# libjxl/libjxl

Hardware: AMD Instinct MI355X
Metric: Mpixels/s decode (VarDCT d1.0, 8K RGB) (higher is better)
Workload: dtype f32

## Files before the change

libjxl_amd/csrc/context.h:

```cpp
#pragma once
#include <stdint.h>
#include <stdio.h>
#include <string.h>

#include <algorithm>
#include <atomic>
#include <chrono>
#include <condition_variable>
#include <memory>
#include <mutex>
#include <vector>

#include "../../include/jxl_hip_codestream.h"
#include "../../include/jxl_hip_entropy.h"
#include "kernels.h"
#include "tile_bins.h"
#include "env_switches.h"

namespace jxlhip {

int Fail(jxlhip_ctx* c, int code, const char* fmt, ...);

#define HIPCHK(c, call)                                                              \
  do {                                                                               \
// ... 291 lines not shown
  int stage_state[kStageSlots] = {0};
  int stage_count = 0;
  int stage_cap = kStageSlots;
  PinnedBuf stage_chunk[kStageSlots / kStageChunk];
  size_t stage_bytes = 0;
  std::mutex stage_mu;
  std::condition_variable stage_cv;
  DevBuf<float> dc_tmp;
  DevBuf<uint8_t> dc_prec;
  DevBuf<uint8_t> host_frame_dev;
  PinnedBuf pinned_frame;
  DevBuf<float> alpha_dev;
  PinnedBuf alpha_host;
  DevBuf<int32_t> qdc_dev;
  StageState st;
  SlotState slots;
  float display_nits = 0.0f;
  uint32_t display_primaries = 0, display_white_point = 0;
  bool seq_open = false;
  uint64_t seq_expect = 0;
  bool generic_filters = false;
  int mfma = -1;
  int fuse = -1;
  DevBuf<uint2> cell_info;
  bool profiling = false;
  std::vector<ProfMarkRec> marks;
};

namespace jxlhip {

inline size_t SparseTableItems(const jxlhip_ctx* c) { return std::min(c->sp_off_host[0].bytes, c->sp_off_host[1].bytes) / 4; }

inline size_t OutSampleBytes(const jxlhip_output_format& o) {
  return o.sample_type == JXLHIP_SAMPLE_U8 ? 1 : (o.sample_type == JXLHIP_SAMPLE_F32 ? 4 : 2);
}
inline size_t OutPixelBytes(uint32_t kind, const jxlhip_output_format& o) {
  if (kind == JXLHIP_OUT_LINEAR_RGB_F32) return 12;
  return kind == JXLHIP_OUT_PACKED ? (size_t)o.num_channels * OutSampleBytes(o) : 0;
}
inline size_t OutPixelBytes(const jxlhip_ctx* c) { return OutPixelBytes(c->p.output_kind, c->p.out_format); }

inline size_t OutCols(const jxlhip_ctx* c) { return c->st.ups.factor > 1 ? c->st.ups.xsize : c->f.xsize; }
inline size_t OutRows(const jxlhip_ctx* c) { return c->st.ups.factor > 1 ? c->st.ups.ysize : c->f.y1 - c->f.y0; }
inline size_t BufCols(const jxlhip_ctx* c) { return c->st.blend.on ? c->st.blend.p.image_xsize : OutCols(c); }
inline size_t BufRows(const jxlhip_ctx* c) { return c->st.blend.on ? c->st.blend.p.image_ysize : OutRows(c); }

// ... 87 lines not shown
```

libjxl_amd/csrc/context.hip:

```cpp
#include <math.h>
#include <stdarg.h>
#include <stdlib.h>
#include <new>

#include "context.h"
#include "dither_pattern.inc"

extern "C" __attribute__((visibility("default"))) void jxlhip_debug_reload_env(void) {
  std::lock_guard<std::mutex> lock(jxlhip_env::g.mu);
  jxlhip_env::LoadLocked();
}

int jxlhip::Fail(jxlhip_ctx* c, int code, const char* fmt, ...) {
  if (c) {
    va_list ap;
    va_start(ap, fmt);
    vsnprintf(c->err, sizeof(c->err), fmt, ap);
    va_end(ap);
  }
  return code;
}

namespace {

// ... 69 lines not shown
  else free(c);
}

int jxlhip_create(int device, jxlhip_ctx** out) { return jxlhip_create_ex(device, nullptr, out); }

int jxlhip_create_ex(int device, const JxlMemoryManagerHip* memory_manager, jxlhip_ctx** out) {
  if (!out) return JXLHIP_ERR_INVALID_ARGUMENT;
  *out = nullptr;
  if (memory_manager && ((memory_manager->alloc == nullptr) != (memory_manager->free == nullptr)))
    return JXLHIP_ERR_INVALID_ARGUMENT;
  int ndev = 0;
  if (hipGetDeviceCount(&ndev) != hipSuccess || ndev <= 0) return JXLHIP_ERR_NO_DEVICE;
  if (device < 0 || device >= ndev) return JXLHIP_ERR_INVALID_ARGUMENT;
  jxlhip_ctx* c = NewCtx(memory_manager);
  if (!c) return JXLHIP_ERR_OUT_OF_MEMORY;
  c->device = device;
  {
    std::lock_guard<std::mutex> lock(jxlhip_env::g.mu);
    jxlhip_env::LoadLocked();
    const jxlhip_env::Switches& s = jxlhip_env::g;
    c->generic_filters = s.generic_filters.load();
    c->sparse_upload = s.sparse_upload.load();
    c->fuse = s.fuse.load();
    c->mfma = s.mfma.load();
    c->prepare_once = s.prepare_once.load();
    const int ss = s.stage_slots.load();
    if (ss != jxlhip_env::Switches::kUnset) {
      const int v = (ss + kStageChunk - 1) / kStageChunk * kStageChunk;
      c->stage_cap = v < kStageSlotsFirst ? kStageSlotsFirst : (v > kStageSlots ? kStageSlots : v);
    }
  }
  auto fail = [&](int code) {
    jxlhip_destroy(c);
    return code;
  };
  if (hipSetDevice(device) != hipSuccess) return fail(JXLHIP_ERR_HIP);
  if (c->own_stream.Create() != hipSuccess) return fail(JXLHIP_ERR_HIP);
  c->stream = c->own_stream;
  for (int i = 0; i < kPoolStreams; i++) {
    if (c->pool[i].Create() != hipSuccess || c->pool_ev[i].Create() != hipSuccess) return fail(JXLHIP_ERR_HIP);
  }
  if (c->frame_ev.Create() != hipSuccess) return fail(JXLHIP_ERR_HIP);
  if (c->counts.Reserve(c, (size_t)kCountStride * kCountBlocks) || c->error_flag.Reserve(c, 2) ||
      c->tables.Reserve(c, kTabFloats) || c->quant_enc.Reserve(c, JXLHIP_NUM_QUANT_TABLES))
    return fail(JXLHIP_ERR_OUT_OF_MEMORY);
  if (hipMemset(c->error_flag, 0, sizeof(int32_t) * 2) != hipSuccess ||
// ... 366 lines not shown
  if (!LaunchFiltersFast(f2, fp, 0, 2, (int)t.kind, c->stream))
    return Fail(c, JXLHIP_ERR_STATE, "EPF1 + EPF2 march refused a frame the EPF0 march accepted");
  return JXLHIP_OK;
}

int LaunchFiltersRows(jxlhip_ctx* c, const OutTarget& t, uint32_t fy0, uint32_t fy1, bool fused = false) {
  const FilterParams& fp = t.fp;
  DevFrame f = c->f;
  f.fy0 = fy0;
  f.fy1 = fy1;
  f.fused = fused ? 1u : 0u;
  f.cell_info = c->cell_info;
  ProfBegin(c);
  if (fused && c->p.lf.epf_iters == 3) {
    bool declined;
    const int rc = LaunchEpf0Then12(c, f, t, true, &declined);
    if (rc) return rc;
    if (declined) return Fail(c, JXLHIP_ERR_STATE, "fused EPF0 kernel refused a frame FusedEpf0Supported accepted");
    ProfMark(c, JXLHIP_KERNEL_FILTERS);
      HIPCHK(c, hipGetLastError());
    return JXLHIP_OK;
  }
  if (fused) {
    if (!LaunchFused(f, fp, (int)c->p.lf.gab, (int)c->p.lf.epf_iters, (int)t.kind, c->stream))
      return Fail(c, JXLHIP_ERR_STATE, "fused kernel refused a frame FusedSupported accepted");
    ProfMark(c, JXLHIP_KERNEL_FUSED);
      HIPCHK(c, hipGetLastError());
    return JXLHIP_OK;
  }
  bool fast = false;
  if (!c->generic_filters && fy1 > fy0 && c->p.lf.epf_iters == 3 && c->planes2) {
    bool declined;
    const int rc = LaunchEpf0Then12(c, f, t, false, &declined);
    if (rc) return rc;
    fast = !declined;
  } else if (!c->generic_filters && fy1 > fy0) {
    fast = LaunchFiltersFast(f, fp, (int)c->p.lf.gab, (int)c->p.lf.epf_iters, (int)t.kind, c->stream);
  }
  if (!fast && LaunchFilters(f, fp, (int)c->p.lf.gab, (int)c->p.lf.epf_iters, (int)t.kind, c->stream) != 0)
    return Fail(c, JXLHIP_ERR_INVALID_ARGUMENT, "unsupported filter configuration");
  ProfMark(c, JXLHIP_KERNEL_FILTERS);
  HIPCHK(c, hipGetLastError());
  return JXLHIP_OK;
}

bool WantFused(const jxlhip_ctx* c, uint32_t kind, const jxlhip_output_format& fmt) {
  const DevFrame& f = c->f;
// ... 479 lines not shown
```

libjxl_amd/csrc/entropy.cc:

```cpp
#include "env_switches.h"
#include <stdlib.h>
#include <string.h>
namespace jxlhip_env {
Switches g;
void LoadLocked() {
  g.wp_general.store(getenv("JXLHIP_WP_GENERAL") != nullptr);
  g.codestream_verbose.store(getenv("JXLHIP_CODESTREAM_VERBOSE") != nullptr);
  g.no_pipeline.store(getenv("JXLHIP_NO_PIPELINE") != nullptr);
  const char* e = getenv("JXLHIP_TEST_RANGE_GROUP");
  g.test_range_group.store(e ? atoll(e) : -1);
  const char* ife = getenv("JXLHIP_MULTI_INTERIOR_FIRST");
  g.multi_interior_first.store(!ife || atoi(ife) != 0 ? 1 : 0);
  auto num = [](const char* v, int unset) { return v ? atoi(v) : unset; };
  auto force = [](const char* v) { return v ? (atoi(v) != 0 ? 1 : 0) : -1; };
  g.fused_pc_rh.store(num(getenv("JXLHIP_FUSED_PC_RH"), 0));
  g.filter_rh.store(num(getenv("JXLHIP_FILTER_RH"), 0));
  g.big_wgs.store(num(getenv("JXLHIP_BIG_WGS"), Switches::kUnset));
  g.r_wgs.store(num(getenv("JXLHIP_R_WGS"), Switches::kUnset));
  g.multi_force_gather.store(getenv("JXLHIP_MULTI_FORCE_GATHER") != nullptr);
  const char* filters = getenv("JXLHIP_FILTERS");
  g.generic_filters.store(filters && !strcmp(filters, "generic"));
  g.sparse_upload.store(num(getenv("JXLHIP_SPARSE_UPLOAD"), 1) != 0);
  g.fuse.store(force(getenv("JXLHIP_FUSE")));
  g.mfma.store(force(getenv("JXLHIP_MFMA")));
  g.stage_slots.store(num(getenv("JXLHIP_STAGE_SLOTS"), Switches::kUnset));
  g.prepare_once.store(num(getenv("JXLHIP_PREPARE_ONCE"), 1) != 0);
  {
    const char* mp = getenv("JXLHIP_MAX_PIXELS");
    char* end = nullptr;
    const unsigned long long v = mp ? strtoull(mp, &end, 10) : 0ull;
    g.max_pixels.store((mp && end != mp && v != 0) ? v : (1ull << 30));
  }
  g.loaded.store(true, std::memory_order_release);
}
}
#include <math.h>
#include <stdlib.h>
#include <string.h>

#include <algorithm>
#include <functional>
#include <memory>
#include <mutex>
#include <new>
#include <vector>

// ... 2568 lines not shown
```

libjxl_amd/csrc/env_switches.h:

```cpp
#ifndef JXLHIP_ENV_SWITCHES_H_
#define JXLHIP_ENV_SWITCHES_H_
#include <atomic>
#include <mutex>

namespace jxlhip_env {
struct Switches {
  std::atomic<bool> loaded{false};
  std::atomic<bool> wp_general{false};
  std::atomic<bool> codestream_verbose{false};
  std::atomic<bool> no_pipeline{false};
  std::atomic<long long> test_range_group{-1};
  std::atomic<int> multi_interior_first{1};
  static constexpr int kUnset = -2147483647 - 1;
  std::atomic<int> fused_pc_rh{0};
  std::atomic<int> filter_rh{0};
  std::atomic<int> big_wgs{kUnset};
  std::atomic<int> r_wgs{kUnset};
  std::atomic<bool> multi_force_gather{false};
  std::atomic<unsigned long long> max_pixels{1ull << 30};
  std::atomic<bool> generic_filters{false};
  std::atomic<bool> sparse_upload{true};
  std::atomic<int> fuse{-1};
  std::atomic<int> mfma{-1};
  std::atomic<int> stage_slots{kUnset};
  std::atomic<bool> prepare_once{true};
  std::mutex mu;
};
extern Switches g;
void LoadLocked();
static inline const Switches& Get() {
  if (!g.loaded.load(std::memory_order_acquire)) {
    std::lock_guard<std::mutex> lock(g.mu);
    if (!g.loaded.load(std::memory_order_relaxed)) LoadLocked();
  }
  return g;
}
}
#endif
```

libjxl_amd/csrc/filters_march.h:

```cpp
#ifndef JXLHIP_FILTERS_MARCH_H_
#define JXLHIP_FILTERS_MARCH_H_

#include "dev_common.h"
#include "emit.h"
#include "kernels.h"

namespace jxlhip {
namespace {

__device__ __forceinline__ int MirrorF(int x, int n) {
  while (x < 0 || x >= n) x = x < 0 ? -x - 1 : 2 * n - 1 - x;
  return x;
}
__device__ __forceinline__ int Mirror1(int y, int n) {
  y = y < 0 ? -y - 1 : y;
  return y >= n ? 2 * n - 1 - y : y;
}

__device__ __forceinline__ uint32_t RowOffset(const DevFrame& f, int y) {
  const uint32_t ry = (uint32_t)(y - f.plane_y0);
  return (ry >> 3) * (f.tile_stride * 256u) + ((ry & 7u) << 5);
}

__device__ __forceinline__ float FromLeft(float v) {
// ... 34 lines not shown
  float y = __builtin_fabsf(d[0].y) * P.ch_scale[0];
  x = __builtin_fmaf(__builtin_fabsf(d[1].x), P.ch_scale[1], x);
  y = __builtin_fmaf(__builtin_fabsf(d[1].y), P.ch_scale[1], y);
  x = __builtin_fmaf(__builtin_fabsf(d[2].x), P.ch_scale[2], x);
  y = __builtin_fmaf(__builtin_fabsf(d[2].y), P.ch_scale[2], y);
  return v2f{Scalar(x), Scalar(y)};
}

__device__ __forceinline__ v2f AddLeftS(v2f acc, v2f p) {
  return v2f{Scalar(FromLeft(p.y) + acc.x), Scalar(acc.y + p.x)};
}
__device__ __forceinline__ v2f AddRightS(v2f acc, v2f p) {
  return v2f{Scalar(acc.x + p.y), Scalar(FromRight(p.x) + acc.y)};
}
__device__ __forceinline__ v2f FmaLeftS(v2f w, v2f p, v2f a) {
  float ax = a.x;
  asm("v_fmac_f32_dpp %0, %1, %2 wave_shr:1 row_mask:0xf bank_mask:0xf bound_ctrl:1" : "+v"(ax) : "v"(p.y), "v"(w.x));
  return v2f{ax, Scalar(__builtin_fmaf(w.y, p.x, a.y))};
}
__device__ __forceinline__ v2f FmaRightS(v2f w, v2f p, v2f a) {
  float ay = a.y;
  asm("v_fmac_f32_dpp %0, %1, %2 wave_shl:1 row_mask:0xf bank_mask:0xf bound_ctrl:1" : "+v"(ay) : "v"(p.x), "v"(w.y));
  return v2f{Scalar(__builtin_fmaf(w.x, p.y, a.x)), ay};
}

struct State {
  v2f x[3][8];
  v2f hs[3][4];
  v2f g[3][4];
  v2f du[4], dl[4];
  v2f pv[4], ph[4];
  v2f e[3][4];
  v2f dv[4];
};

struct Lane {
  uint32_t byte_off;
  bool sel0, sel1;
  int gx;
  bool out0, out1;
  v2f mul;
  v2f mul2;
  bool fix_left, fix_right_even, fix_right_odd;
  uint32_t sx4;
  uint32_t out_off;
  const float __attribute__((address_space(3))) * dither;
  const float __attribute__((address_space(3))) * slab;
};

enum RowSource : int { SRC_PLANES = 0, SRC_LDS = 1, SRC_LINEAR = 2 };
template <int SRC>
__device__ __forceinline__ uint32_t SrcRowOffset(const DevFrame& f, int y) {
  if constexpr (SRC == SRC_LINEAR) return (uint32_t)(y - f.plane_y0) * f.linear_stride;
  else return RowOffset(f, y);
}
static constexpr int kSlabCols = 128;
static constexpr int kSlabPlaneFloats = 8 * kSlabCols;
static constexpr int kSlabBytes = 3 * kSlabPlaneFloats * 4;

template <bool EDGE>
__device__ __forceinline__ v2f LdsPair(const Lane& L, int c, int row) {
  typedef v2f __attribute__((address_space(3))) * P2;
  const v2f v = *(P2)(L.slab + c * kSlabPlaneFloats + row * kSlabCols);
  if constexpr (!EDGE) return v;
  return v2f{L.sel0 ? v.y : v.x, L.sel1 ? v.y : v.x};
}

template <bool EDGE>
__device__ __forceinline__ v2f LoadPair(const char* rowp, Lane& L) {
  const v2f v = *(const v2f*)(rowp + L.byte_off);
  if constexpr (!EDGE) return v;
  return v2f{L.sel0 ? v.y : v.x, L.sel1 ? v.y : v.x};
}

typedef float f4u __attribute__((ext_vector_type(4), aligned(4)));
typedef float f2u __attribute__((ext_vector_type(2), aligned(4)));

struct XybConsts {
  v2f b01, b23, b45;
  v2f m0a, m1a, m2a;
};
// ... 114 lines not shown
    } else if (L.out1) {
      __builtin_nontemporal_store(o.p1.y, dst + 3);
      __builtin_nontemporal_store(o.p2.x, dst + 4);
      __builtin_nontemporal_store(o.p2.y, dst + 5);
    }
  } else {
    LaneOffset(L.out_off);
#pragma unroll
    for (int c = 0; c < 3; c++) {
      float* d = (float*)(out_row + (size_t)c * P.out_plane_stride * 4 + L.out_off);
      if (EDGE ? (L.out0 && L.out1) : L.out0) {
        __builtin_nontemporal_store(f2u{v[c].x, v[c].y}, (f2u*)d);
      } else if (!EDGE) {
      } else if (L.out0) {
        __builtin_nontemporal_store(v[c].x, d);
      } else if (L.out1) {
        __builtin_nontemporal_store(v[c].y, d + 1);
      }
    }
  }
}

enum StepKnown : int { kStepGeneric = 0, kStepInterior = 1, kStepEmit = 2, kStepFirst = 4 };
template <int GAB, int EPF, int OUTK, int FMT, int PH, bool EDGE, int SRC = SRC_PLANES, int KNOWN = kStepGeneric>
__device__ __forceinline__ void Step(State& s, int r, const DevFrame& f, const FilterParams& P,
                                     Lane& L, int prefetch_last_row, int y_begin, int y_end,
                                     float& inv_sigma_blk, float& inv_sigma_blk2, char* out_row, const XybConsts& K,
                                     int slab_y0 = 0, float sigma_pre = 0.0f, float sigma_prev = 0.0f) {
  constexpr int S0 = PH & 3, S1 = (PH + 3) & 3, S2 = (PH + 2) & 3;
  constexpr int X0 = PH & 7, X1 = (PH + 7) & 7, X2 = (PH + 6) & 7, X3 = (PH + 5) & 7;
  const int H = (int)f.ysize;
  if constexpr (SRC == SRC_LDS) {
    if constexpr (PH < 7) {
      const int nrow = (KNOWN & kStepInterior) ? PH + 1 : Mirror1(r + 1, H) - slab_y0;
#pragma unroll
      for (int c = 0; c < 3; c++) s.x[c][(PH + 1) & 7] = LdsPair<EDGE>(L, c, nrow);
    }
  } else if constexpr (PH % kBurst == 0) {
    LaneOffset(L.byte_off);
#pragma unroll
    for (int b = 0; b < kBurst; b++) {
      int pr = r + kAhead + b;
      pr = pr > prefetch_last_row ? prefetch_last_row : pr;
      const uint32_t off = SrcRowOffset<SRC>(f, Mirror1(pr, H));
#pragma unroll
      for (int c = 0; c < 3; c++) s.x[c][(PH + kAhead + b) & 7] = LoadPair<EDGE>((const char*)f.xyb[c] + off, L);
    }
  }
  v2f gq[3];
  if constexpr (GAB) {
#pragma unroll
    for (int c = 0; c < 3; c++) {
      const v2f cur = s.x[c][X0];
      s.hs[c][S0] = v2f{Scalar(FromLeft(cur.y) + cur.y), Scalar(FromRight(cur.x) + cur.x)};
      const v2f sum1 = s.hs[c][S1] + (s.x[c][X2] + cur);
      const v2f sum2 = s.hs[c][S2] + s.hs[c][S0];
      gq[c] = Fma2(sum2, P.gab_w[c][2], Fma2(sum1, P.gab_w[c][1], s.x[c][X1] * P.gab_w[c][0]));
    }
  } else {
#pragma unroll
    for (int c = 0; c < 3; c++) gq[c] = s.x[c][X0];
  }
  constexpr int Q0 = GAB ? S1 : S0;
  constexpr int Q1 = (Q0 + 3) & 3, Q2 = (Q0 + 2) & 3, Q3 = (Q0 + 1) & 3;
  const int q = GAB ? r - 1 : r;
  v2f gq1[3], gq2[3], gq3[3];
#pragma unroll
  for (int c = 0; c < 3; c++) {
    gq1[c] = GAB ? s.g[c][Q1] : s.x[c][X1];
    gq2[c] = GAB ? s.g[c][Q2] : s.x[c][X2];
    gq3[c] = GAB ? s.g[c][Q3] : s.x[c][X3];
  }
  v2f outv[3];
  int o;
  if constexpr (EPF) {
    {
      v2f dvert[3], dhor[3];
#pragma unroll
      for (int c = 0; c < 3; c++) {
        dvert[c] = gq1[c] - gq[c];
        dhor[c] = v2f{Scalar(FromLeft(gq[c].y) - gq[c].x), Scalar(gq[c].x - gq[c].y)};
        if constexpr (GAB) s.g[c][Q0] = gq[c];
      }
      s.du[Q0] = AbsScaleSum(dvert, P);
      s.dl[Q0] = AbsScaleSum(dhor, P);
    }
    {
      const v2f du_c = s.du[Q1], dl_c = s.dl[Q1];
      v2f v = AddLeftS(s.du[Q2], du_c);
      v = v + du_c;
      v = AddRightS(v, du_c);
      s.pv[Q1] = v + s.du[Q0];
      v2f h = AddLeftS(s.dl[Q2], dl_c);
      h = h + dl_c;
      h = AddRightS(h, dl_c);
      s.ph[Q1] = h + s.dl[Q0];
    }
    o = q - 2;
    const float kMinSigma = -3.90524291751269967465540850526868f;
    constexpr bool kInt = (KNOWN & kStepInterior) != 0;
    static_assert(!kInt || SRC == SRC_LDS, "kStepInterior: the fused kernel's march");
    constexpr int kIy = (PH - GAB - 2 + 16) & 7;
    if (kInt ? (kIy == 0 || (EPF == 2 && (KNOWN & kStepFirst) && kIy == 7)) : ((o & 7) == 0 || o == y_begin - (EPF == 2 ? 1 : 0))) {
      float is = (kInt ? kIy == 0 : (o & 7) == 0) ? sigma_pre : sigma_prev;
      if constexpr (SRC != SRC_LDS) {
// ... 103 lines not shown
```

libjxl_amd/csrc/fused_pc.h:

```cpp
#ifndef JXLHIP_FUSED_PC_H_
#define JXLHIP_FUSED_PC_H_

#include <stdlib.h>

#include <type_traits>

#include "blocks_common.h"
#include "env_switches.h"
#include "filters_march.h"

static constexpr int kProducerPrio = 3;

namespace jxlhip {

namespace {

typedef __attribute__((address_space(3))) float LdsF;
typedef __attribute__((address_space(3))) uint32_t LdsU;

static constexpr int kFusedHalo = 8;
static constexpr int kFusedUse = kSlabCols - 2 * kFusedHalo;

typedef const DevFrame __attribute__((address_space(4))) * FrameArgs;
__device__ __forceinline__ FrameArgs Fresh(FrameArgs q) {
// ... 250 lines not shown
#pragma unroll
  for (int c = 0; c < 3; c++) {
    k.coef[c] = (const char*)f->coeffs[c];
    k.dc[c] = (const char*)f->dc[c];
    k.xyb[c] = f->xyb[c];
  }
  k.cell_info = (const char*)f->cell_info;
  k.inv_sigma = (const char*)f->inv_sigma;
  k.xsb = (int)f->xsb;
  k.tile_stride = f->tile_stride;
  k.plane_tile_row0 = f->plane_y0 >> 3;
  k.inv_global_scale = f->inv_global_scale;
  k.x_dm = f->x_dm;
  k.b_dm = f->b_dm;
  k.cfl_base_x = f->cfl_base_x;
  k.cfl_base_b = f->cfl_base_b;
  k.color_scale = f->color_scale;
#pragma unroll
  for (int i = 0; i < 4; i++) k.bias[i] = f->biases[i];
  return k;
}
__device__ __forceinline__ u4v AsmLoad4S(const char* base, uint32_t off) {
  u4v r;
  asm volatile("global_load_dwordx4 %0, %1, %2" : "=v"(r) : "v"(off), "s"(base) : "memory");
  return r;
}
__device__ __forceinline__ u2v AsmLoad2S(const char* base, uint32_t off) {
  u2v r;
  asm volatile("global_load_dwordx2 %0, %1, %2" : "=v"(r) : "v"(off), "s"(base) : "memory");
  return r;
}
__device__ __forceinline__ uint32_t AsmLoad1S(const char* base, uint32_t off) {
  uint32_t r;
  asm volatile("global_load_dword %0, %1, %2" : "=v"(r) : "v"(off), "s"(base) : "memory");
  return r;
}

__device__ __forceinline__ void PcLanded(PcNext& n) { asm volatile("" : "+v"(n.ci), "+v"(n.sg)); }
__device__ __forceinline__ void PcLanded(PcGroupRegs& R) {
#pragma unroll
  for (int s = 0; s < 2; s++)
#pragma unroll
    for (int c = 0; c < 3; c++) asm volatile("" : "+v"(R.st[s].rows[c]), "+v"(R.st[s].dcv[c]));
}

__device__ __forceinline__ void PcRequest(const PcK& K, PcNext& n, int nb, int bc0) {
  const int lane = threadIdx.x & 63;
  int col = bc0 + (lane & 15);
  col = col < 0 ? 0 : (col >= K.xsb ? K.xsb - 1 : col);
  const uint32_t cell = (uint32_t)(nb * K.xsb + col);
  n.nb = nb;
  n.ci = AsmLoad2S(K.cell_info, cell * 8u);
  n.sg = AsmLoad1S(K.inv_sigma, cell * 4u);
}

__device__ __forceinline__ void PcIssue(const PcK& K, LdsU* list, const PcNext& n, int bc0, PcGroupRegs& R) {
  const int lane = threadIdx.x & 63;
// ... 93 lines not shown
          const float sc = c == 0 ? sx : sb;
          const float cc = c == 0 ? x_cc : b_cc;
          unpack(T.rows[c], q);
#pragma unroll
          for (int k = 0; k < 8; k++) {
            const float d = AdjustQuantBias(q[k], c == 0 ? bias0 : bias2, bias3) * (tab[c][k] * sc);
            v[k] = __builtin_fmaf(cc, vy[k], d);
          }
        }
        if (j == 0) v[0] = __uint_as_float(T.dcv[c]);
        IdctReg<8>(v);
        Transpose8Lanes(v, bit3);
        IdctReg<8>(v);
        LdsF* dst = slab + c * kSlabPlaneFloats + j * kSlabCols + T.cell * 8;
        if (valid) {
          *(P4)dst = f4v{v[0], v[1], v[2], v[3]};
          *(P4)(dst + 4) = f4v{v[4], v[5], v[6], v[7]};
        }
      }
    }
  }
}

template <int HX>
__device__ __forceinline__ void ProducePC2(FrameArgs fa, StripLds* w, int bc0, int y_begin, int y_end, int nb_last) {
  const int lane = threadIdx.x & 63;
  const int r_first = HX ? y_begin - 8 : y_begin;
  const int G = PcGroups<HX>(y_begin, y_end);
  const PcK K = MakePcK(fa);
  float tab[3][8];
  {
    const int j = lane >> 3;
#pragma unroll
    for (int c = 0; c < 3; c++) {
      const float4 t0 = *(const float4*)(fa->dequant + c * 64 + j * 8);
      const float4 t1 = *(const float4*)(fa->dequant + c * 64 + j * 8 + 4);
      tab[c][0] = t0.x, tab[c][1] = t0.y, tab[c][2] = t0.z, tab[c][3] = t0.w;
      tab[c][4] = t1.x, tab[c][5] = t1.y, tab[c][6] = t1.z, tab[c][7] = t1.w;
    }
  }
  LdsU* list = (LdsU*)w->list[0];
  auto group_nb = [&](int g) { return GroupBlockRow(r_first + 8 * (g < G ? g : G - 1), nb_last); };
  PcGroupRegs A, B;
  PcNext n0, n1;
  uint32_t sg_a = 0, sg_b = 0;
  PcRequest(K, n0, group_nb(0), bc0);
  asm volatile("s_waitcnt vmcnt(0)" ::: "memory");
  PcLanded(n0);
  PcIssue(K, list, n0, bc0, A);
  sg_a = n0.sg;
  PcRequest(K, n1, group_nb(1), bc0);
  asm volatile("s_waitcnt vmcnt(0)" ::: "memory");
  PcLanded(A);
  PcLanded(n1);
  auto body = [&](int g, PcGroupRegs& CUR, PcGroupRegs& NXT, uint32_t& sg_cur, uint32_t& sg_nxt, PcNext& nn) {
    LdsF* slab = (LdsF*)w->slab[(g & 1)];
    PcDmaPlanes(K, slab, CUR.mp, CUR.nb, bc0);
    PcIssue(K, list, nn, bc0, NXT);
    sg_nxt = nn.sg;
    PcRequest(K, nn, group_nb(g + 2), bc0);
    PcDecode(K, slab, CUR, tab);
    if (lane < 16) ((LdsU*)w->sigma[g & 1])[lane] = sg_cur;
    PcBarrierProducer();
    PcLanded(NXT);
    PcLanded(nn);
  };
  for (int g = 0; g < G; g += 2) {
    body(g, A, B, sg_a, sg_b, n1);
    if (g + 1 < G) body(g + 1, B, A, sg_b, sg_a, n1);
  }
}

int FusedRowsPC(unsigned strips, unsigned rows, unsigned per_cu = kPcPerCu) {
  const int forced = jxlhip_env::Get().fused_pc_rh.load(std::memory_order_relaxed);
  if (forced > 0) return (forced + 7) & ~7;
  return ChunkRows(strips, rows, DeviceCus() * per_cu, 16, 1024, 8, 6 + 16);
}

}
}
#endif
```

libjxl_amd/csrc/kernels.h:

```cpp
#ifndef JXLHIP_KERNELS_H_
#define JXLHIP_KERNELS_H_

#include "dev_common.h"

namespace jxlhip {

struct WorkLists {
  WorkItem* list[kNumClasses];
  uint32_t* count;
};

struct SharpLut {
  float v[8];
};

struct FilterParams {
  float gab_w[3][3];
  float ch_scale[3];
  float sm[3], bsm[3];
  float opsin_bias[3];
  float cbrt_bias[3];
  float minv[9];
  float xyb_bias[6];
  float mcol[3][4];
// ... 14 lines not shown
                   const SharpLut& lut, hipStream_t st);
void LaunchBlocks(const DevFrame& f, const WorkLists& wl, uint32_t cells, const float* wc,
                  const float* resample, hipStream_t st, const FilterParams* emit = nullptr);
int LaunchFilters(const DevFrame& f, const FilterParams& p, int gab, int epf_iters,
                  int output_kind, hipStream_t st);

bool LaunchFiltersFast(const DevFrame& f, const FilterParams& p, int gab, int epf_iters,
                       int output_kind, hipStream_t st);
bool FastFixedFormat(const jxlhip_output_format& o);

bool LaunchEpf0(const DevFrame& f, const FilterParams& p, int gab, float* const dst[3], hipStream_t st);

void LaunchExpandSparse(const uint8_t* sparse, const uint32_t* offsets, int16_t* dense, uint32_t g0, uint32_t n, hipStream_t st);

bool LaunchOrient(const void* src, size_t src_stride, uint32_t xsize, uint32_t ysize, uint32_t bytes_per_pixel,
                  uint32_t orientation, void* dst, size_t dst_stride, hipStream_t st);

void MfmaDct32Constants(float* host );
void MfmaDct16Constants(float* host );
void LaunchMfma32(const DevFrame& f, const WorkLists& wl, uint32_t cells, hipStream_t st, const FilterParams* emit = nullptr);
void LaunchMfma16(const DevFrame& f, const WorkLists& wl, uint32_t cells, hipStream_t st);

bool FusedSupported(const DevFrame& f, int gab, int epf_iters, int output_kind);
bool LaunchFused(const DevFrame& f, const FilterParams& p, int gab, int epf_iters, int output_kind,
                 hipStream_t st);
bool FusedEpf0Supported(const DevFrame& f, int gab);
bool LaunchFusedEpf0(const DevFrame& f, const FilterParams& p, int gab, float* const dst[3], hipStream_t st);
unsigned DeviceCus();
inline int ChunkRows(unsigned wgx, unsigned rows, unsigned resident, int first, int last, int step, int overhead) {
  int best = 64;
  double best_cost = 1e30;
  for (int rh = first; rh <= last; rh += step) {
    const unsigned wgs = wgx * ((rows + rh - 1) / rh);
    const unsigned gens = (wgs + resident - 1) / resident;
    const double cost = (double)gens * (rh + overhead);
    if (cost < best_cost) {
      best_cost = cost;
      best = rh;
    }
  }
  return best;
}

constexpr uint32_t kNoiseSegFills = 128;
constexpr uint32_t kNoiseSegs = (3u * 256u * 16u + kNoiseSegFills - 1) / kNoiseSegFills;
constexpr uint32_t kNoiseJumpWords = 128 * 4;
struct NoiseArgs {
// ... 144 lines not shown
```

libjxl_amd/csrc/kernels_fused.hip:

```cpp
#include "fused_pc.h"

namespace jxlhip {

namespace {

template <int GAB, int EPF, int OUTK, int FMT, bool EDGE, bool INTERIOR, int NB = 2>
__device__ __forceinline__ void MarchPC(const DevFrame& f, const FilterParams& P, Lane& L, StripLdsT<NB>* w, int bc0,
                                        int y_begin, int y_end) {
  constexpr int HX = MarchGeom<GAB, EPF>::HX;
  constexpr int KI = INTERIOR ? (int)kStepInterior : 0;
  constexpr int KE = INTERIOR ? (int)(kStepInterior | kStepEmit) : 0;
  constexpr int KF = INTERIOR ? (int)kStepFirst : 0;
  const int H = (int)f.ysize;
  const int r_first = HX ? y_begin - 8 : y_begin;
  const int r_last = y_end + HX - 1;
  const int nb_last = (H - 1) >> 3;
  const int G = PcGroups<HX>(y_begin, y_end);
  State s;
#pragma unroll
  for (int k = 0; k < 8; k++)
#pragma unroll
    for (int c = 0; c < 3; c++) s.x[c][k] = v2f{0.0f, 0.0f};
#pragma unroll
  for (int k = 0; k < 4; k++) {
#pragma unroll
    for (int c = 0; c < 3; c++) {
      s.hs[c][k] = v2f{0.0f, 0.0f};
      s.g[c][k] = v2f{0.0f, 0.0f};
      s.e[c][k] = v2f{0.0f, 0.0f};
    }
    s.du[k] = v2f{0.0f, 0.0f};
    s.dl[k] = v2f{0.0f, 0.0f};
    s.pv[k] = v2f{0.0f, 0.0f};
    s.ph[k] = v2f{0.0f, 0.0f};
    s.dv[k] = v2f{0.0f, 0.0f};
  }
  float inv_sigma_blk = -1.0f, inv_sigma_blk2 = -1.0f;
  float sigma_last = -1.0f;
  const XybConsts KC = MakeXybConsts(P);
  const size_t out_row_bytes = OUTK == JXLHIP_OUT_XYB_PLANAR ? P.out_stride * 4 : P.out_stride;
  char* out_row = (char*)P.out + (ptrdiff_t)(r_first - HX - (int)f.y0) * (ptrdiff_t)out_row_bytes;
  const float __attribute__((address_space(3)))* const slab0 = L.slab;
  const LdsF* sig0 = (const LdsF*)w->sigma[0] + ((int)(L.sx4 >> 2) - bc0);
  int i = 0;
  auto enter_group = [&](int g) -> float {
    const int b = NB == 2 ? (g & 1) : g % NB;
    L.slab = slab0 + b * (3 * kSlabPlaneFloats);
    return EPF ? sig0[b * 16] : 0.0f;
  };
#define JXLHIP_PSTEPK(K, KN)                                                                                          \
  Step<GAB, EPF, OUTK, FMT, K, EDGE, SRC_LDS, KN>(s, r + K, f, P, L, 0, y_begin, y_end, inv_sigma_blk,         \
                                                  inv_sigma_blk2, out_row, KC, slab_y0, sigma_pre, sigma_prev);       \
  out_row += out_row_bytes
#define JXLHIP_PGROUP(KLOW, KHIGH)                                                       \
  {                                                                                      \
    const int slab_y0 = GroupBlockRow(r, nb_last) * 8;                                   \
    const float sigma_prev = sigma_last;                                                 \
    const float sigma_pre = enter_group(i);                                              \
    sigma_last = sigma_pre;                                                              \
    {                                                                                    \
      const int row0 = INTERIOR ? 0 : Mirror1(r, H) - slab_y0;                           \
      _Pragma("unroll") for (int c = 0; c < 3; c++) s.x[c][0] = LdsPair<EDGE>(L, c, row0); \
    }                                                                                    \
    JXLHIP_PSTEPK(0, (0 < HX ? (KLOW) : (KHIGH)));                                       \
    JXLHIP_PSTEPK(1, (1 < HX ? (KLOW) : (KHIGH)));                                       \
    JXLHIP_PSTEPK(2, (2 < HX ? (KLOW) : (KHIGH)));                                       \
    JXLHIP_PSTEPK(3, (3 < HX ? (KLOW) : (KHIGH)));                                       \
    JXLHIP_PSTEPK(4, (KHIGH));                                                           \
    JXLHIP_PSTEPK(5, (KHIGH));                                                           \
    JXLHIP_PSTEPK(6, (KHIGH));                                                           \
    JXLHIP_PSTEPK(7, (KHIGH));                                                           \
    i++;                                                                                 \
  }
  PcBarrierMarch();
  if constexpr (HX > 0) {
    const int r = r_first;
    const int slab_y0 = GroupBlockRow(r, nb_last) * 8;
    const float sigma_prev = sigma_last;
    const float sigma_pre = enter_group(i);
    sigma_last = sigma_pre;
    {
      const int row0 = INTERIOR ? 8 - HX : Mirror1(r + 8 - HX, H) - slab_y0;
#pragma unroll
      for (int c = 0; c < 3; c++) s.x[c][8 - HX] = LdsPair<EDGE>(L, c, row0);
    }
    out_row += (8 - HX) * out_row_bytes;
    if constexpr (HX >= 4) { JXLHIP_PSTEPK(4, KI); }
    if constexpr (HX >= 3) { JXLHIP_PSTEPK(5, KI); }
    if constexpr (HX >= 2) { JXLHIP_PSTEPK(6, KI); }
    JXLHIP_PSTEPK(7, KI);
    i++;
    PcBarrierMarch();
  }
  int r = HX ? y_begin : r_first;
  if constexpr (INTERIOR) {
    JXLHIP_PGROUP(KI | KF, KE | KF)
    if (i < G) PcBarrierMarch();
    for (r += 8; r < y_end; r += 8) {
      JXLHIP_PGROUP(KE, KE)
      if (i < G) PcBarrierMarch();
    }
  } else {
    for (; r_last - r >= HX; r += 8) {
      JXLHIP_PGROUP(0, 0)
      if (i < G) PcBarrierMarch();
    }
  }
  if (HX > 0 && (INTERIOR || r <= r_last)) {
    const int slab_y0 = GroupBlockRow(r, nb_last) * 8;
    const float sigma_prev = sigma_last;
    const float sigma_pre = enter_group(i);
    sigma_last = sigma_pre;
    {
      const int row0 = INTERIOR ? 0 : Mirror1(r, H) - slab_y0;
#pragma unroll
      for (int c = 0; c < 3; c++) s.x[c][0] = LdsPair<EDGE>(L, c, row0);
    }
    JXLHIP_PSTEPK(0, KE);
    if constexpr (HX >= 2) { JXLHIP_PSTEPK(1, KE); }
    if constexpr (HX >= 3) { JXLHIP_PSTEPK(2, KE); }
    if constexpr (HX >= 4) { JXLHIP_PSTEPK(3, KE); }
  }
#undef JXLHIP_PGROUP
#undef JXLHIP_PSTEPK
}

template <int GAB, int EPF, int OUTK, int FMT, typename CT>
__global__ __launch_bounds__(128, kPcWaves) void k_fused_pc(DevFrame f, FilterParams P, int RH, int strips, int nwg) {
  __shared__ StripLds lds;
  const int lane = threadIdx.x & 63;
  const int wave = (int)(threadIdx.x >> 6);
  const float __attribute__((address_space(3)))* dither_lds = nullptr;
  if constexpr (OUTK == JXLHIP_OUT_PACKED) {
    __shared__ float s_dither[1024];
    if (P.fmt.sample_type == JXLHIP_SAMPLE_U8) {
      for (int i = threadIdx.x; i < 1024; i += 128) s_dither[i] = P.dither[i];
      __syncthreads();
    }
    dither_lds = (const float __attribute__((address_space(3)))*)s_dither;
  }
  const int per = (int)gridDim.x >> 3;
  const int logical = ((int)blockIdx.x & 7) * per + ((int)blockIdx.x >> 3);
  if (logical >= nwg) return;
  const int strip = logical % strips, chunk = logical / strips;
  const int W = (int)f.xsize;
  const int x_first = strip * kFusedUse;
  const int y_begin = (int)f.fy0 + chunk * RH;
  const int y_end = min(y_begin + RH, (int)f.fy1);
  if (x_first >= W || y_begin >= y_end) return;
  const int x0 = x_first - kFusedHalo;
  const int bc0 = x0 >> 3;
  const FrameArgs fa = (FrameArgs)__builtin_amdgcn_kernarg_segment_ptr();
  if (wave == 1) {
    __builtin_amdgcn_s_setprio(kProducerPrio);
    if constexpr (sizeof(CT) == 2) ProducePC2<MarchGeom<GAB, EPF>::HX>(fa, &lds, bc0, y_begin, y_end, ((int)f.ysize - 1) >> 3);
    else
      ProducePC<MarchGeom<GAB, EPF>::HX, CT>(fa, &lds, bc0, y_begin, y_end, ((int)f.ysize - 1) >> 3);
    return;
  }
  Lane L;
  L.gx = x0 + 2 * lane;
  L.dither = dither_lds;
  const int m0 = MirrorF(L.gx, W), m1 = MirrorF(L.gx + 1, W);
  int base = (m0 & ~1) - x0;
  base = base < 0 ? 0 : (base > kSlabCols - 2 ? kSlabCols - 2 : base);
  L.sel0 = m0 & 1;
  L.sel1 = m1 & 1;
  L.byte_off = 0;
  L.slab = (const float __attribute__((address_space(3)))*)lds.slab[0] + base;
  const bool edge = x0 < 0 || x0 + kSlabCols > W;
  const bool lane_in = lane >= kFusedHalo / 2 && lane < 64 - kFusedHalo / 2;
  L.out0 = lane_in && L.gx < W;
  L.out1 = lane_in && L.gx + 1 < W;
  const int gxc = L.gx < 0 ? 0 : (L.gx >= W ? W - 1 : L.gx);
  L.sx4 = (uint32_t)(gxc >> 3) * 4u;
  L.out_off = (uint32_t)(L.gx < 0 ? 0 : L.gx) * (OUTK == JXLHIP_OUT_LINEAR_RGB_F32 ? 12u : 4u);
  const int ix = gxc & 7;
  L.mul = v2f{ix == 0 ? P.bsm[1] : P.sm[1], ix == 6 ? P.bsm[1] : P.sm[1]};
  L.mul2 = v2f{ix == 0 ? P.bsm[2] : P.sm[2], ix == 6 ? P.bsm[2] : P.sm[2]};
  L.fix_left = L.gx == -2;
  L.fix_right_even = L.gx == W;
  L.fix_right_odd = L.gx == W - 1;
  const bool interior = (y_begin & 7) == 0 && ((y_end - y_begin) & 7) == 0 && y_begin >= 8 &&
                        y_end + 8 <= (int)f.ysize;
  if (interior) {
    if (edge) MarchPC<GAB, EPF, OUTK, FMT, true, true>(f, P, L, &lds, bc0, y_begin, y_end);
    else MarchPC<GAB, EPF, OUTK, FMT, false, true>(f, P, L, &lds, bc0, y_begin, y_end);
  } else {
    if (edge) MarchPC<GAB, EPF, OUTK, FMT, true, false>(f, P, L, &lds, bc0, y_begin, y_end);
    else MarchPC<GAB, EPF, OUTK, FMT, false, false>(f, P, L, &lds, bc0, y_begin, y_end);
  }
}

template <int GAB, int EPF, int OUTK, int FMT = -1>
void LaunchFusedPcT(const DevFrame& f, const FilterParams& p, hipStream_t st) {
  const unsigned strips = (f.xsize + kFusedUse - 1) / kFusedUse;
  const int RH = FusedRowsPC(strips, f.fy1 - f.fy0);
  const unsigned nwg = strips * ((f.fy1 - f.fy0 + RH - 1) / RH);
  const dim3 grid((nwg + 7) & ~7u);
  if (f.coeff_type == JXLHIP_COEFF_I16)
    hipLaunchKernelGGL((k_fused_pc<GAB, EPF, OUTK, FMT, int16_t>), grid, dim3(128), 0, st, f, p, RH, (int)strips, (int)nwg);
  else
    hipLaunchKernelGGL((k_fused_pc<GAB, EPF, OUTK, FMT, int32_t>), grid, dim3(128), 0, st, f, p, RH, (int)strips, (int)nwg);
}

}

bool FusedSupported(const DevFrame& f, int gab, int epf_iters, int output_kind) {
  (void)gab;
  if (epf_iters > 2) return false;
  if (output_kind == JXLHIP_OUT_PACKED) return false;
  if (f.xsize < 16 || f.ysize < 16) return false;
  const uint32_t tail = f.ysize & 7u;
  if (tail >= 1 && tail <= 3) return false;
  if ((f.fy0 & 7u) != 0) return false;
  if ((uint64_t)f.plane_tile_rows * f.tile_stride * 256u >= (1ull << 32)) return false;
  if ((uint64_t)f.xsg * f.ysg * f.coef_stride64 * 64u * (f.coeff_type == JXLHIP_COEFF_I16 ? 2u : 4u) >= (1ull << 32)) return false;
  return true;
}

bool LaunchFused(const DevFrame& f, const FilterParams& p, int gab, int epf_iters, int output_kind, hipStream_t st) {
  if (!FusedSupported(f, gab, epf_iters, output_kind)) return false;
#define JXLHIP_FUSED_PCX(G, E)                                    \
  if (gab == G && epf_iters == E) {                               \
    if (output_kind == 0) LaunchFusedPcT<G, E, 0>(f, p, st);      \
    else LaunchFusedPcT<G, E, 1>(f, p, st);                       \
    return true;                                                  \
  }
  JXLHIP_FUSED_PCX(1, 1)
  JXLHIP_FUSED_PCX(0, 0)
  JXLHIP_FUSED_PCX(0, 1)
  JXLHIP_FUSED_PCX(1, 0)
  JXLHIP_FUSED_PCX(0, 2)
  JXLHIP_FUSED_PCX(1, 2)
#undef JXLHIP_FUSED_PCX
  return false;
}

}
```

Before: 121,300.

## Add opt-in producer-side Gaborish pass in fused PC kernel; pad global loads with s_nop

Adds an env-gated mode (JXLHIP_FUSED_PREGAB, off by default) in which the producer wave applies the Gaborish smoothing to each decoded slab in LDS, so the consumer march skips its own Gaborish work and reads pre-filtered rows with a remapped slab index. This is meant to move filter arithmetic off the consumer wave and onto the producer, at the cost of an extra full vmcnt wait and LDS rewrites in the producer. Separately, every inline-asm global load in the fused producer now starts with an s_nop 4, which changes instruction timing on the default path as well.

```diff
diff --git a/libjxl_amd/csrc/context.h b/libjxl_amd/csrc/context.h
--- a/libjxl_amd/csrc/context.h
+++ b/libjxl_amd/csrc/context.h
@@ -337,6 +337,7 @@
   bool generic_filters = false;
   int mfma = -1;
   int fuse = -1;
+  int fused_pregab = -1;
   DevBuf<uint2> cell_info;
   bool profiling = false;
   std::vector<ProfMarkRec> marks;
diff --git a/libjxl_amd/csrc/context.hip b/libjxl_amd/csrc/context.hip
--- a/libjxl_amd/csrc/context.hip
+++ b/libjxl_amd/csrc/context.hip
@@ -115,6 +115,7 @@
     c->generic_filters = s.generic_filters.load();
     c->sparse_upload = s.sparse_upload.load();
     c->fuse = s.fuse.load();
+    c->fused_pregab = s.fused_pregab.load();
     c->mfma = s.mfma.load();
     c->prepare_once = s.prepare_once.load();
     const int ss = s.stage_slots.load();
@@ -527,7 +528,7 @@
     return JXLHIP_OK;
   }
   if (fused) {
-    if (!LaunchFused(f, fp, (int)c->p.lf.gab, (int)c->p.lf.epf_iters, (int)t.kind, c->stream))
+    if (!LaunchFused(f, fp, (int)c->p.lf.gab, (int)c->p.lf.epf_iters, (int)t.kind, c->fused_pregab, c->stream))
       return Fail(c, JXLHIP_ERR_STATE, "fused kernel refused a frame FusedSupported accepted");
     ProfMark(c, JXLHIP_KERNEL_FUSED);
       HIPCHK(c, hipGetLastError());
diff --git a/libjxl_amd/csrc/entropy.cc b/libjxl_amd/csrc/entropy.cc
--- a/libjxl_amd/csrc/entropy.cc
+++ b/libjxl_amd/csrc/entropy.cc
@@ -22,6 +22,7 @@
   g.generic_filters.store(filters && !strcmp(filters, "generic"));
   g.sparse_upload.store(num(getenv("JXLHIP_SPARSE_UPLOAD"), 1) != 0);
   g.fuse.store(force(getenv("JXLHIP_FUSE")));
+  g.fused_pregab.store(force(getenv("JXLHIP_FUSED_PREGAB")));
   g.mfma.store(force(getenv("JXLHIP_MFMA")));
   g.stage_slots.store(num(getenv("JXLHIP_STAGE_SLOTS"), Switches::kUnset));
   g.prepare_once.store(num(getenv("JXLHIP_PREPARE_ONCE"), 1) != 0);
diff --git a/libjxl_amd/csrc/env_switches.h b/libjxl_amd/csrc/env_switches.h
--- a/libjxl_amd/csrc/env_switches.h
+++ b/libjxl_amd/csrc/env_switches.h
@@ -21,6 +21,7 @@
   std::atomic<bool> generic_filters{false};
   std::atomic<bool> sparse_upload{true};
   std::atomic<int> fuse{-1};
+  std::atomic<int> fused_pregab{-1};
   std::atomic<int> mfma{-1};
   std::atomic<int> stage_slots{kUnset};
   std::atomic<bool> prepare_once{true};
diff --git a/libjxl_amd/csrc/filters_march.h b/libjxl_amd/csrc/filters_march.h
--- a/libjxl_amd/csrc/filters_march.h
+++ b/libjxl_amd/csrc/filters_march.h
@@ -80,6 +80,16 @@
   float ay = a.y;
   asm("v_fmac_f32_dpp %0, %1, %2 wave_shl:1 row_mask:0xf bank_mask:0xf bound_ctrl:1" : "+v"(ay) : "v"(p.x), "v"(w.y));
   return v2f{Scalar(__builtin_fmaf(w.x, p.y, a.x)), ay};
+}
+
+__device__ __forceinline__ v2f GabHs(v2f cur) {
+  return v2f{Scalar(FromLeft(cur.y) + cur.y), Scalar(FromRight(cur.x) + cur.x)};
+}
+__device__ __forceinline__ v2f GabRow(v2f above, v2f centre, v2f below, v2f hs_above, v2f hs_centre, v2f hs_below,
+                                      const float* w) {
+  const v2f sum1 = hs_centre + (above + below);
+  const v2f sum2 = hs_above + hs_below;
+  return Fma2(sum2, w[2], Fma2(sum1, w[1], centre * w[0]));
 }
 
 struct State {
@@ -115,6 +125,12 @@
 static constexpr int kSlabCols = 128;
 static constexpr int kSlabPlaneFloats = 8 * kSlabCols;
 static constexpr int kSlabBytes = 3 * kSlabPlaneFloats * 4;
+
+template <int PREGAB>
+__device__ __forceinline__ int SlabRowOfStep(int r, int H, int slab_y0) {
+  if constexpr (PREGAB) return (Mirror1(r - 1, H) + 1 - slab_y0) & 7;
+  else return Mirror1(r, H) - slab_y0;
+}
 
 template <bool EDGE>
 __device__ __forceinline__ v2f LdsPair(const Lane& L, int c, int row) {
@@ -275,17 +291,19 @@
 }
 
 enum StepKnown : int { kStepGeneric = 0, kStepInterior = 1, kStepEmit = 2, kStepFirst = 4 };
-template <int GAB, int EPF, int OUTK, int FMT, int PH, bool EDGE, int SRC = SRC_PLANES, int KNOWN = kStepGeneric>
+template <int GAB, int EPF, int OUTK, int FMT, int PH, bool EDGE, int SRC = SRC_PLANES, int KNOWN = kStepGeneric,
+          int PREGAB = 0>
 __device__ __forceinline__ void Step(State& s, int r, const DevFrame& f, const FilterParams& P,
                                      Lane& L, int prefetch_last_row, int y_begin, int y_end,
                                      float& inv_sigma_blk, float& inv_sigma_blk2, char* out_row, const XybConsts& K,
                                      int slab_y0 = 0, float sigma_pre = 0.0f, float sigma_prev = 0.0f) {
   constexpr int S0 = PH & 3, S1 = (PH + 3) & 3, S2 = (PH + 2) & 3;
   constexpr int X0 = PH & 7, X1 = (PH + 7) & 7, X2 = (PH + 6) & 7, X3 = (PH + 5) & 7;
+  static_assert(!PREGAB || (GAB && SRC == SRC_LDS), "PREGAB: Gaborish applied by the fused kernel's producing wave");
   const int H = (int)f.ysize;
   if constexpr (SRC == SRC_LDS) {
     if constexpr (PH < 7) {
-      const int nrow = (KNOWN & kStepInterior) ? PH + 1 : Mirror1(r + 1, H) - slab_y0;
+      const int nrow = (KNOWN & kStepInterior) ? PH + 1 : SlabRowOfStep<PREGAB>(r + 1, H, slab_y0);
 #pragma unroll
       for (int c = 0; c < 3; c++) s.x[c][(PH + 1) & 7] = LdsPair<EDGE>(L, c, nrow);
     }
@@ -301,14 +319,11 @@
     }
   }
   v2f gq[3];
-  if constexpr (GAB) {
+  if constexpr (GAB && !PREGAB) {
 #pragma unroll
     for (int c = 0; c < 3; c++) {
-      const v2f cur = s.x[c][X0];
-      s.hs[c][S0] = v2f{Scalar(FromLeft(cur.y) + cur.y), Scalar(FromRight(cur.x) + cur.x)};
-      const v2f sum1 = s.hs[c][S1] + (s.x[c][X2] + cur);
-      const v2f sum2 = s.hs[c][S2] + s.hs[c][S0];
-      gq[c] = Fma2(sum2, P.gab_w[c][2], Fma2(sum1, P.gab_w[c][1], s.x[c][X1] * P.gab_w[c][0]));
+      s.hs[c][S0] = GabHs(s.x[c][X0]);
+      gq[c] = GabRow(s.x[c][X2], s.x[c][X1], s.x[c][X0], s.hs[c][S2], s.hs[c][S1], s.hs[c][S0], P.gab_w[c]);
     }
   } else {
 #pragma unroll
@@ -320,9 +335,9 @@
   v2f gq1[3], gq2[3], gq3[3];
 #pragma unroll
   for (int c = 0; c < 3; c++) {
-    gq1[c] = GAB ? s.g[c][Q1] : s.x[c][X1];
-    gq2[c] = GAB ? s.g[c][Q2] : s.x[c][X2];
-    gq3[c] = GAB ? s.g[c][Q3] : s.x[c][X3];
+    gq1[c] = (GAB && !PREGAB) ? s.g[c][Q1] : s.x[c][X1];
+    gq2[c] = (GAB && !PREGAB) ? s.g[c][Q2] : s.x[c][X2];
+    gq3[c] = (GAB && !PREGAB) ? s.g[c][Q3] : s.x[c][X3];
   }
   v2f outv[3];
   int o;
@@ -333,7 +348,7 @@
       for (int c = 0; c < 3; c++) {
         dvert[c] = gq1[c] - gq[c];
         dhor[c] = v2f{Scalar(FromLeft(gq[c].y) - gq[c].x), Scalar(gq[c].x - gq[c].y)};
-        if constexpr (GAB) s.g[c][Q0] = gq[c];
+        if constexpr (GAB && !PREGAB) s.g[c][Q0] = gq[c];
       }
       s.du[Q0] = AbsScaleSum(dvert, P);
       s.dl[Q0] = AbsScaleSum(dhor, P);
diff --git a/libjxl_amd/csrc/fused_pc.h b/libjxl_amd/csrc/fused_pc.h
--- a/libjxl_amd/csrc/fused_pc.h
+++ b/libjxl_amd/csrc/fused_pc.h
@@ -296,17 +296,17 @@
 }
 __device__ __forceinline__ u4v AsmLoad4S(const char* base, uint32_t off) {
   u4v r;
-  asm volatile("global_load_dwordx4 %0, %1, %2" : "=v"(r) : "v"(off), "s"(base) : "memory");
+  asm volatile("s_nop 4\n\tglobal_load_dwordx4 %0, %1, %2" : "=v"(r) : "v"(off), "s"(base) : "memory");
   return r;
 }
 __device__ __forceinline__ u2v AsmLoad2S(const char* base, uint32_t off) {
   u2v r;
-  asm volatile("global_load_dwordx2 %0, %1, %2" : "=v"(r) : "v"(off), "s"(base) : "memory");
+  asm volatile("s_nop 4\n\tglobal_load_dwordx2 %0, %1, %2" : "=v"(r) : "v"(off), "s"(base) : "memory");
   return r;
 }
 __device__ __forceinline__ uint32_t AsmLoad1S(const char* base, uint32_t off) {
   uint32_t r;
-  asm volatile("global_load_dword %0, %1, %2" : "=v"(r) : "v"(off), "s"(base) : "memory");
+  asm volatile("s_nop 4\n\tglobal_load_dword %0, %1, %2" : "=v"(r) : "v"(off), "s"(base) : "memory");
   return r;
 }
 
@@ -446,8 +446,56 @@
   }
 }
 
-template <int HX>
-__device__ __forceinline__ void ProducePC2(FrameArgs fa, StripLds* w, int bc0, int y_begin, int y_end, int nb_last) {
+template <bool EDGE>
+__device__ __forceinline__ void GabPass(const FilterParams& P, const Lane& L0, int buffer, int nb, int rows, bool refill,
+                                        v2f (&up2)[3], v2f (&up1)[3]) {
+  Lane L;
+  L.slab = L0.slab + buffer * (3 * kSlabPlaneFloats);
+  L.sel0 = L0.sel0, L.sel1 = L0.sel1;
+  L.out0 = L0.out0, L.out1 = L0.out1;
+  v2f hs2[3], hs1[3];
+#pragma unroll
+  for (int c = 0; c < 3; c++) {
+    hs2[c] = GabHs(up2[c]);
+    hs1[c] = GabHs(up1[c]);
+  }
+#pragma unroll
+  for (int k = 0; k < 8; k++) {
+    v2f cur[3];
+#pragma unroll
+    for (int c = 0; c < 3; c++) cur[c] = k < rows ? LdsPair<EDGE>(L, c, k) : up1[c];
+    if (k == 0 && nb == 0) {
+#pragma unroll
+      for (int c = 0; c < 3; c++) {
+        up1[c] = cur[c];
+        hs1[c] = GabHs(cur[c]);
+      }
+    }
+#pragma unroll
+    for (int c = 0; c < 3; c++) {
+      const v2f below = (k == 0 && refill) ? up1[c] : cur[c];
+      const v2f hs0 = GabHs(below);
+      const v2f g = GabRow(up2[c], up1[c], below, hs2[c], hs1[c], hs0, P.gab_w[c]);
+      typedef v2f __attribute__((address_space(3))) * P2;
+      LdsF* dst = (LdsF*)L.slab + c * kSlabPlaneFloats + k * kSlabCols;
+      if constexpr (!EDGE) {
+        *(P2)dst = g;
+      } else if (L.out1) {
+        *(P2)dst = g;
+      } else if (L.out0) {
+        *dst = g.x;
+      }
+      up2[c] = up1[c];
+      hs2[c] = hs1[c];
+      up1[c] = cur[c];
+      hs1[c] = (k == 0 && refill) ? GabHs(cur[c]) : hs0;
+    }
+  }
+}
+
+template <int HX, int PREGAB = 0, bool EDGE = false>
+__device__ __forceinline__ void ProducePC2(FrameArgs fa, StripLds* w, int bc0, int y_begin, int y_end, int nb_last,
+                                           const FilterParams* P = nullptr, const Lane* L = nullptr) {
   const int lane = threadIdx.x & 63;
   const int r_first = HX ? y_begin - 8 : y_begin;
   const int G = PcGroups<HX>(y_begin, y_end);
@@ -468,6 +516,9 @@
   PcGroupRegs A, B;
   PcNext n0, n1;
   uint32_t sg_a = 0, sg_b = 0;
+  v2f up2[3] = {v2f{0.0f, 0.0f}, v2f{0.0f, 0.0f}, v2f{0.0f, 0.0f}}, up1[3] = {v2f{0.0f, 0.0f}, v2f{0.0f, 0.0f}, v2f{0.0f, 0.0f}};
+  int nb_prev = -1;
+  const int H = PREGAB ? (int)fa->ysize : 0;
   PcRequest(K, n0, group_nb(0), bc0);
   asm volatile("s_waitcnt vmcnt(0)" ::: "memory");
   PcLanded(n0);
@@ -484,6 +535,11 @@
     sg_nxt = nn.sg;
     PcRequest(K, nn, group_nb(g + 2), bc0);
     PcDecode(K, slab, CUR, tab);
+    if constexpr (PREGAB) {
+      asm volatile("s_waitcnt vmcnt(0)" ::: "memory");
+      GabPass<EDGE>(*P, *L, g & 1, CUR.nb, H - 8 * CUR.nb, CUR.nb == nb_prev && CUR.nb == nb_last, up2, up1);
+      nb_prev = CUR.nb;
+    }
     if (lane < 16) ((LdsU*)w->sigma[g & 1])[lane] = sg_cur;
     PcBarrierProducer();
     PcLanded(NXT);
diff --git a/libjxl_amd/csrc/kernels.h b/libjxl_amd/csrc/kernels.h
--- a/libjxl_amd/csrc/kernels.h
+++ b/libjxl_amd/csrc/kernels.h
@@ -60,7 +60,7 @@
 void LaunchMfma16(const DevFrame& f, const WorkLists& wl, uint32_t cells, hipStream_t st);
 
 bool FusedSupported(const DevFrame& f, int gab, int epf_iters, int output_kind);
-bool LaunchFused(const DevFrame& f, const FilterParams& p, int gab, int epf_iters, int output_kind,
+bool LaunchFused(const DevFrame& f, const FilterParams& p, int gab, int epf_iters, int output_kind, int pregab,
                  hipStream_t st);
 bool FusedEpf0Supported(const DevFrame& f, int gab);
 bool LaunchFusedEpf0(const DevFrame& f, const FilterParams& p, int gab, float* const dst[3], hipStream_t st);
diff --git a/libjxl_amd/csrc/kernels_fused.hip b/libjxl_amd/csrc/kernels_fused.hip
--- a/libjxl_amd/csrc/kernels_fused.hip
+++ b/libjxl_amd/csrc/kernels_fused.hip
@@ -4,7 +4,7 @@
 
 namespace {
 
-template <int GAB, int EPF, int OUTK, int FMT, bool EDGE, bool INTERIOR, int NB = 2>
+template <int GAB, int EPF, int OUTK, int FMT, bool EDGE, bool INTERIOR, int PREGAB = 0, int NB = 2>
 __device__ __forceinline__ void MarchPC(const DevFrame& f, const FilterParams& P, Lane& L, StripLdsT<NB>* w, int bc0,
                                         int y_begin, int y_end) {
   constexpr int HX = MarchGeom<GAB, EPF>::HX;
@@ -49,7 +49,7 @@
     return EPF ? sig0[b * 16] : 0.0f;
   };
 #define JXLHIP_PSTEPK(K, KN)                                                                                          \
-  Step<GAB, EPF, OUTK, FMT, K, EDGE, SRC_LDS, KN>(s, r + K, f, P, L, 0, y_begin, y_end, inv_sigma_blk,         \
+  Step<GAB, EPF, OUTK, FMT, K, EDGE, SRC_LDS, KN, PREGAB>(s, r + K, f, P, L, 0, y_begin, y_end, inv_sigma_blk,         \
                                                   inv_sigma_blk2, out_row, KC, slab_y0, sigma_pre, sigma_prev);       \
   out_row += out_row_bytes
 #define JXLHIP_PGROUP(KLOW, KHIGH)                                                       \
@@ -59,7 +59,7 @@
     const float sigma_pre = enter_group(i);                                              \
     sigma_last = sigma_pre;                                                              \
     {                                                                                    \
-      const int row0 = INTERIOR ? 0 : Mirror1(r, H) - slab_y0;                           \
+      const int row0 = INTERIOR ? 0 : SlabRowOfStep<PREGAB>(r, H, slab_y0);              \
       _Pragma("unroll") for (int c = 0; c < 3; c++) s.x[c][0] = LdsPair<EDGE>(L, c, row0); \
     }                                                                                    \
     JXLHIP_PSTEPK(0, (0 < HX ? (KLOW) : (KHIGH)));                                       \
@@ -80,7 +80,7 @@
     const float sigma_pre = enter_group(i);
     sigma_last = sigma_pre;
     {
-      const int row0 = INTERIOR ? 8 - HX : Mirror1(r + 8 - HX, H) - slab_y0;
+      const int row0 = INTERIOR ? 8 - HX : SlabRowOfStep<PREGAB>(r + 8 - HX, H, slab_y0);
 #pragma unroll
       for (int c = 0; c < 3; c++) s.x[c][8 - HX] = LdsPair<EDGE>(L, c, row0);
     }
@@ -112,7 +112,7 @@
     const float sigma_pre = enter_group(i);
     sigma_last = sigma_pre;
     {
-      const int row0 = INTERIOR ? 0 : Mirror1(r, H) - slab_y0;
+      const int row0 = INTERIOR ? 0 : SlabRowOfStep<PREGAB>(r, H, slab_y0);
 #pragma unroll
       for (int c = 0; c < 3; c++) s.x[c][0] = LdsPair<EDGE>(L, c, row0);
     }
@@ -125,8 +125,9 @@
 #undef JXLHIP_PSTEPK
 }
 
-template <int GAB, int EPF, int OUTK, int FMT, typename CT>
+template <int GAB, int EPF, int OUTK, int FMT, typename CT, int PREGAB = 0>
 __global__ __launch_bounds__(128, kPcWaves) void k_fused_pc(DevFrame f, FilterParams P, int RH, int strips, int nwg) {
+  static_assert(!PREGAB || (GAB && sizeof(CT) == 2), "PREGAB: a Gaborish stage list on the pipelined producer");
   __shared__ StripLds lds;
   const int lane = threadIdx.x & 63;
   const int wave = (int)(threadIdx.x >> 6);
@@ -151,24 +152,33 @@
   const int x0 = x_first - kFusedHalo;
   const int bc0 = x0 >> 3;
   const FrameArgs fa = (FrameArgs)__builtin_amdgcn_kernarg_segment_ptr();
-  if (wave == 1) {
-    __builtin_amdgcn_s_setprio(kProducerPrio);
-    if constexpr (sizeof(CT) == 2) ProducePC2<MarchGeom<GAB, EPF>::HX>(fa, &lds, bc0, y_begin, y_end, ((int)f.ysize - 1) >> 3);
-    else
-      ProducePC<MarchGeom<GAB, EPF>::HX, CT>(fa, &lds, bc0, y_begin, y_end, ((int)f.ysize - 1) >> 3);
-    return;
-  }
   Lane L;
   L.gx = x0 + 2 * lane;
-  L.dither = dither_lds;
   const int m0 = MirrorF(L.gx, W), m1 = MirrorF(L.gx + 1, W);
   int base = (m0 & ~1) - x0;
   base = base < 0 ? 0 : (base > kSlabCols - 2 ? kSlabCols - 2 : base);
   L.sel0 = m0 & 1;
   L.sel1 = m1 & 1;
-  L.byte_off = 0;
   L.slab = (const float __attribute__((address_space(3)))*)lds.slab[0] + base;
   const bool edge = x0 < 0 || x0 + kSlabCols > W;
+  if (wave == 1) {
+    __builtin_amdgcn_s_setprio(kProducerPrio);
+    constexpr int HX = MarchGeom<GAB, EPF>::HX;
+    const int nb_last = ((int)f.ysize - 1) >> 3;
+    if constexpr (PREGAB) {
+      L.out0 = L.gx >= 0 && L.gx < W;
+      L.out1 = L.gx >= 0 && L.gx + 1 < W;
+      if (edge) ProducePC2<HX, 1, true>(fa, &lds, bc0, y_begin, y_end, nb_last, &P, &L);
+      else ProducePC2<HX, 1, false>(fa, &lds, bc0, y_begin, y_end, nb_last, &P, &L);
+    } else if constexpr (sizeof(CT) == 2) {
+      ProducePC2<HX>(fa, &lds, bc0, y_begin, y_end, nb_last);
+    } else {
+      ProducePC<HX, CT>(fa, &lds, bc0, y_begin, y_end, nb_last);
+    }
+    return;
+  }
+  L.dither = dither_lds;
+  L.byte_off = 0;
   const bool lane_in = lane >= kFusedHalo / 2 && lane < 64 - kFusedHalo / 2;
   L.out0 = lane_in && L.gx < W;
   L.out1 = lane_in && L.gx + 1 < W;
@@ -184,20 +194,26 @@
   const bool interior = (y_begin & 7) == 0 && ((y_end - y_begin) & 7) == 0 && y_begin >= 8 &&
                         y_end + 8 <= (int)f.ysize;
   if (interior) {
-    if (edge) MarchPC<GAB, EPF, OUTK, FMT, true, true>(f, P, L, &lds, bc0, y_begin, y_end);
-    else MarchPC<GAB, EPF, OUTK, FMT, false, true>(f, P, L, &lds, bc0, y_begin, y_end);
+    if (edge) MarchPC<GAB, EPF, OUTK, FMT, true, true, PREGAB>(f, P, L, &lds, bc0, y_begin, y_end);
+    else MarchPC<GAB, EPF, OUTK, FMT, false, true, PREGAB>(f, P, L, &lds, bc0, y_begin, y_end);
   } else {
-    if (edge) MarchPC<GAB, EPF, OUTK, FMT, true, false>(f, P, L, &lds, bc0, y_begin, y_end);
-    else MarchPC<GAB, EPF, OUTK, FMT, false, false>(f, P, L, &lds, bc0, y_begin, y_end);
+    if (edge) MarchPC<GAB, EPF, OUTK, FMT, true, false, PREGAB>(f, P, L, &lds, bc0, y_begin, y_end);
+    else MarchPC<GAB, EPF, OUTK, FMT, false, false, PREGAB>(f, P, L, &lds, bc0, y_begin, y_end);
   }
 }
 
 template <int GAB, int EPF, int OUTK, int FMT = -1>
-void LaunchFusedPcT(const DevFrame& f, const FilterParams& p, hipStream_t st) {
+void LaunchFusedPcT(const DevFrame& f, const FilterParams& p, bool pregab, hipStream_t st) {
   const unsigned strips = (f.xsize + kFusedUse - 1) / kFusedUse;
   const int RH = FusedRowsPC(strips, f.fy1 - f.fy0);
   const unsigned nwg = strips * ((f.fy1 - f.fy0 + RH - 1) / RH);
   const dim3 grid((nwg + 7) & ~7u);
+  if constexpr (GAB != 0) {
+    if (pregab && f.coeff_type == JXLHIP_COEFF_I16) {
+      hipLaunchKernelGGL((k_fused_pc<GAB, EPF, OUTK, FMT, int16_t, 1>), grid, dim3(128), 0, st, f, p, RH, (int)strips, (int)nwg);
+      return;
+    }
+  }
   if (f.coeff_type == JXLHIP_COEFF_I16)
     hipLaunchKernelGGL((k_fused_pc<GAB, EPF, OUTK, FMT, int16_t>), grid, dim3(128), 0, st, f, p, RH, (int)strips, (int)nwg);
   else
@@ -219,12 +235,14 @@
   return true;
 }
 
-bool LaunchFused(const DevFrame& f, const FilterParams& p, int gab, int epf_iters, int output_kind, hipStream_t st) {
+bool LaunchFused(const DevFrame& f, const FilterParams& p, int gab, int epf_iters, int output_kind, int pregab,
+                 hipStream_t st) {
   if (!FusedSupported(f, gab, epf_iters, output_kind)) return false;
+  const bool pg = pregab > 0;
 #define JXLHIP_FUSED_PCX(G, E)                                    \
   if (gab == G && epf_iters == E) {                               \
-    if (output_kind == 0) LaunchFusedPcT<G, E, 0>(f, p, st);      \
-    else LaunchFusedPcT<G, E, 1>(f, p, st);                       \
+    if (output_kind == 0) LaunchFusedPcT<G, E, 0>(f, p, pg, st);  \
+    else LaunchFusedPcT<G, E, 1>(f, p, pg, st);                   \
     return true;                                                  \
   }
   JXLHIP_FUSED_PCX(1, 1)
```

Measured after the change: 120,600. No clear change (-0.6%).
